# YuemingJin/STswinCL

Hardware: AMD Instinct MI355X
Metric: input frames/s, TswinPlus fwd+bwd+Adam, 4-frame 512x512 clips (higher is better)
Workload: dtype bf16; 1 GPU; BASELINE.json configs[1]: TswinPlus(12) seg train step, 4 clips/GPU x T=4 frames x 3x512x512, swin res (64,64), OHEM-CE, Adam; T=4 because the reference asserts it (swin_512.py:313); clips_per_gpu=4, frames_per_clip=4, parallelism=dp1, graph_requested=True

## Files before the change

include/stswin_hip.h:

```cpp
#ifndef STSWIN_HIP_H
#define STSWIN_HIP_H
#ifdef __cplusplus
extern "C" {
#endif

#define STSWIN_GF_GELU 1
#define STSWIN_GF_RESID 2
#define STSWIN_GF_MUL_DGELU 4
#define STSWIN_GF_OUT_F32 8
#define STSWIN_GF_ACCUM 16
#define STSWIN_GF_RELU 32
#define STSWIN_GF_MUL_R 8192
#define STSWIN_GF_C2_DGELU 16384
#define STSWIN_GF_CS_PARTIAL 32768
#define STSWIN_GF_CS_SQ 65536
#define STSWIN_GF_TAPSKIP (1 << 29)
#define STSWIN_GF_BIG 128
#define STSWIN_GF_MID 512
#define STSWIN_GF_NOPIPE 1024
#define STSWIN_GF_HALF 2048
#define STSWIN_GF_M32PP (1u << 31)
#define STSWIN_GF_W4R (1 << 30)
#define STSWIN_GF_ROT 4096
#define STSWIN_GF_NOBIG 256
// ... 181 lines not shown
                        void* out, long ldo, unsigned char* arg, int frames, int H, int W, int C, int groups, int unit_rows, void* stream);
int stswin_rows_broadcast(int dtype, const float* v, void* out, long ldo, int M, int C, int groups, float scale,
                          int accumulate, void* stream);
int stswin_bilinear(int dtype, const void* in, long ldi, void* out, long ldo, int frames, int h, int w, int H, int W, int C,
                    int backward, void* stream);
int stswin_logits_upsample(int dtype, const void* tokens, long ldt, void* nchw, int frames, int h, int w, int H, int W,
                           int nc, int backward, void* stream);

int stswin_ce_fwd(int dtype, const void* logits, const long* labels, float* loss, float* stats, int frames, long HW, int nc,
                  int ignore_index, float thresh, void* stream);
#define STSWIN_OHEM_WORK_BYTES (3 * 2048 * 12 + 48)
int stswin_ohem_select(const float* loss, long n, long n_min, float thresh, const float* stats, void* work, long work_bytes,
                       float* value, float* sel, void* stream);
int stswin_ce_bwd(int dtype, const void* logits, const long* labels, const float* loss, const float* sel,
                  const float* gscale, void* dlogits, int frames, long HW, int nc, int ignore_index, void* stream);

int stswin_contrast_fwd(int dtype, const void* Q, long ldq, const void* const* K5, long ldk, const int* lq,
                        const int* const* lk5, float* pos, float* all, int N, int HW, int C, void* stream);

int stswin_contrast_bank_fwd(int dtype, const void* Q, long ldq, const int* lq, int M, int C, int q_sets, int q_block,
                             const void* bank, long ldb, const int* lb, int maps, int seg, int bank_block, int groups,
                             const int* gmap , float inv_tau, float* pos, float* all,
                             float* rowmax, float* lse, float* workspace, long workspace_floats, void* stream);
int stswin_contrast_bank_fwd_unit(int dtype, const void* Q, long ldq, const int* lq, int M, int C, int q_sets, int q_block,
                             const void* bank, long ldb, const int* lb, int maps, int seg, int bank_block, int groups,
                             const int* gmap , float inv_tau, float* pos, float* all,
                             float* rowmax, float* lse, float* workspace, long workspace_floats, void* stream);
int stswin_contrast_class_sums(int dtype, const void* bank, long ldb, const int* lb, int maps, int seg, int bank_block, int C,
                               int ncls, float* ksum, float* scratch , void* stream);
long stswin_contrast_class_sums_scratch(int maps, int seg, int bank_block, int C, int ncls);
int stswin_contrast_bank_dq(const float* dpos, const float* dneg, const float* cnt, const int* lq, const float* ksum, float* dq,
                            long lddq, int M, int C, int q_sets, int q_block, int seg, int bank_block, int ncls, int groups, const int* gmap,
                            void* stream);

int stswin_rownorm_scatter(int dtype, const void* X, long ldx, void* Y, long ldy, float* inv, int R, int C, int views, int HW, int samples,
                           void* stream);
int stswin_rownorm_scatter_bwd(int dtype, const void* X, long ldx, const float* inv, const float* dY, long lddy, void* dX, long lddx, int R,
                               int C, int views, int HW, int samples, void* stream);
int stswin_labels_resize(const float* const* masks, int maps, int N, int Hs, int Ws, int h, int w, int* lb, void* stream);
int stswin_label_counts(const int* lq, const int* lb, int M, int maps, int seg, int q_sets, int q_block, int bank_block, int ncls, int groups,
                        const int* gmap, int* hist, float* cnt, void* stream);
int stswin_pair_loss(const float* pos, const float* all, const float* cnt, int M, int groups, int q_sets, int visible, float* loss,
                     void* stream);
int stswin_pair_loss_bwd(const float* pos, const float* all, const float* cnt, const float* dloss, int M, int groups, int q_sets, int visible,
                         float* dpos, float* dneg, void* stream);

int stswin_upsample_argmax(int dtype, const void* logits, unsigned char* labels, const long* gt, int* counts, int frames,
                           int nc, int h, int w, int H, int W, void* stream);
int stswin_upsample_argmax_cm(int dtype, const void* logits, unsigned char* labels, const long* gt, unsigned long long* cm, int ncm,
                              int align_corners, int frames, int nc, int h, int w, int H, int W, void* stream);

int stswin_frame_ingest(const unsigned char* in, unsigned char* tmp, float* out, int n, int Hs, int Ws, int H, int W,
                        const int* hbounds, const int* hcoef, int hksize, const int* vbounds, const int* vcoef, int vksize,
                        const float* lut, void* stream);
int stswin_frame_ingest_planes(const unsigned char* in, unsigned char* tmp, float* out, int n, int Hs, int Ws, int H, int W,
                               const int* hbounds, const int* hcoef, int hksize, const int* vbounds, const int* vcoef, int vksize,
                               const float* lut, void* stream);
int stswin_clip_assemble(int dtype, void* ring, const void* fresh, void* clips, const int* table, int B, int n_store, int slots,
                         int n_fresh, long frame_elems, void* stream);

long stswin_augment_crop_table_stride(int Hc, int Wc, int ksize);
int stswin_augment_crop(const unsigned char* frames, const unsigned char* labels, unsigned char* tmp, unsigned char* crop,
                        unsigned char* label_crop, const int* table, long table_stride, int ksize, int B, int T, int Hs, int Ws,
                        int Hc, int Wc, void* stream);
long stswin_augment_finish_table_stride(int Hc, int Wc);
int stswin_augment_finish(const unsigned char* crop, const unsigned char* label_crop, float* images, long* labels_out,
                          const int* table, long table_stride, const float* lut, int lut_planes, const long* label_lut, int B,
                          int T, int Hc, int Wc, void* stream);

int stswin_multi_tensor(int mode, int count, void* const* p, const void* const* g, void* const* m, void* const* v,
                        const int* n, float lr, float b1, float b2, float eps, float wd, float c1, float c2, void* stream);

int stswin_multi_tensor_lars(int count, void* const* p, const void* const* g, void* const* m, const int* n, float* norms,
                             long norms_floats, float lr, float momentum, float wd, float trust_coef, float eps, int first, int adaptive,
                             void* stream);

int stswin_optim_tick(int kind, int* counter, float* hyper, double a, double b, void* stream);
int stswin_multi_tensor_dev(int mode, int count, void* const* p, const void* const* g, void* const* m, void* const* v, const int* n,
                            const float* hyper, float b1, float b2, float eps, float wd, int first, void* stream);
int stswin_multi_tensor_lars_dev(int count, void* const* p, const void* const* g, void* const* m, const int* n, float* norms,
                                 long norms_floats, const float* hyper, float momentum, float wd, float trust_coef, float eps, int first,
                                 int adaptive, void* stream);

int stswin_selftest(float* out, int which, void* stream);
long stswin_calib_mfma(int waves_per_cu, int iters, float* sink, void* stream);
int stswin_calib_copy(const void* src, void* dst, long bytes, void* stream);
int stswin_proxy_collective(const void* src, void* dst, long bytes, int workgroups, int passes, void* stream);

#ifdef __cplusplus
}
#endif
#endif
```

stswincl_amd/csrc/optim.hip:

```cpp
#include "common.h"

#define MT_MAX 48
#define MT_CHUNK 8192

struct MTArgs {
  float* p[MT_MAX];
  const float* g[MT_MAX];
  float* m[MT_MAX];
  float* v[MT_MAX];
  int n[MT_MAX];
  int count;
  float lr, b1, b2, eps, wd, c1, c2;
  int mode;
  const float* norms;
  float trust;
  const float* hyper;
};

__global__ void optim_tick_kernel(int kind, int* __restrict__ counter, float* __restrict__ hyper, double a, double b) {
  if (threadIdx.x != 0 || blockIdx.x != 0) return;
  if (kind == 0) {
    const int t = counter[0] + 1;
    counter[0] = t;
    hyper[1] = (float)(1.0 - pow(a, (double)t));
    hyper[2] = (float)sqrt(1.0 - pow(b, (double)t));
  } else {
    const int k = counter[0];
    counter[0] = k + 1;
    hyper[3] = (float)(1.0 - (1.0 - a) * (cos(3.141592653589793 * (double)k / b) + 1.0) / 2.0);
  }
}

extern "C" int stswin_optim_tick(int kind, int* counter, float* hyper, double a, double b, void* stream) {
  if (kind < 0 || kind > 1 || !counter || !hyper) return -1604;
  hipLaunchKernelGGL(optim_tick_kernel, dim3(1), dim3(64), 0, (hipStream_t)stream, kind, counter, hyper, a, b);
  STSWIN_CHECK_LAUNCH();
  return 0;
}

__global__ __launch_bounds__(256) void mt_norms_kernel(MTArgs a, float* __restrict__ norms) {
  int b = blockIdx.x, t = 0;
  for (; t < a.count; ++t) {
    const int nb = (a.n[t] + MT_CHUNK - 1) / MT_CHUNK;
    if (b < nb) break;
    b -= nb;
  }
  if (t >= a.count) return;
  const int n = a.n[t];
  const float* __restrict__ p = a.p[t];
  const float* __restrict__ g = a.g[t];
  const int base = b * MT_CHUNK, end = min(n, base + MT_CHUNK);
  float sp = 0.f, sg = 0.f;
  for (int i = base + threadIdx.x * 4; i < end; i += 256 * 4) {
    const int cnt = min(4, end - i);
    if (cnt == 4 && ((((uintptr_t)(p + i)) | ((uintptr_t)(g + i))) & 15) == 0) {
      const f32x4 pv = *(const f32x4*)(p + i), gv = *(const f32x4*)(g + i);
#pragma unroll
      for (int e = 0; e < 4; ++e) { const float gr = gv[e] + a.wd * pv[e]; sp += pv[e] * pv[e]; sg += gr * gr; }
    } else {
      for (int e = 0; e < cnt; ++e) { const float pv = p[i + e], gr = g[i + e] + a.wd * pv; sp += pv * pv; sg += gr * gr; }
    }
  }
  sp = wave_sum(sp);
  sg = wave_sum(sg);
  __shared__ float fold[4][2];
  if ((threadIdx.x & 63) == 0) { fold[threadIdx.x >> 6][0] = sp; fold[threadIdx.x >> 6][1] = sg; }
  __syncthreads();
  if (threadIdx.x == 0) {
    norms[2 * (long)blockIdx.x] = fold[0][0] + fold[1][0] + fold[2][0] + fold[3][0];
    norms[2 * (long)blockIdx.x + 1] = fold[0][1] + fold[1][1] + fold[2][1] + fold[3][1];
  }
}

__global__ __launch_bounds__(256) void mt_norms_fold_kernel(MTArgs a, const float* __restrict__ part, float* __restrict__ norms) {
  const int t = blockIdx.x;
  long b0 = 0;
  for (int i = 0; i < t; ++i) b0 += (a.n[i] + MT_CHUNK - 1) / MT_CHUNK;
  const int nb = (a.n[t] + MT_CHUNK - 1) / MT_CHUNK;
  float sp = 0.f, sg = 0.f;
  for (int b = threadIdx.x; b < nb; b += 256) { sp += part[2 * (b0 + b)]; sg += part[2 * (b0 + b) + 1]; }
  sp = wave_sum(sp);
  sg = wave_sum(sg);
  __shared__ float fold[4][2];
  if ((threadIdx.x & 63) == 0) { fold[threadIdx.x >> 6][0] = sp; fold[threadIdx.x >> 6][1] = sg; }
  __syncthreads();
  if (threadIdx.x == 0) {
    norms[2 * t] = fold[0][0] + fold[1][0] + fold[2][0] + fold[3][0];
    norms[2 * t + 1] = fold[0][1] + fold[1][1] + fold[2][1] + fold[3][1];
  }
}

__global__ __launch_bounds__(256) void multi_tensor_kernel(MTArgs a) {
  int b = blockIdx.x, t = 0;
  for (; t < a.count; ++t) {
    const int nb = (a.n[t] + MT_CHUNK - 1) / MT_CHUNK;
    if (b < nb) break;
    b -= nb;
  }
  if (t >= a.count) return;
  const int n = a.n[t];
  float* __restrict__ p = a.p[t];
  const float* __restrict__ g = a.g[t];
  float* __restrict__ m = a.m[t];
  float* __restrict__ v = a.v[t];
  const int base = b * MT_CHUNK;
  const int end = min(n, base + MT_CHUNK);
  float lr = a.lr, b1 = a.b1, c1 = a.c1, c2 = a.c2;
  if (a.hyper) {
    if (a.mode == 2) b1 = a.hyper[3];
    else lr = a.hyper[0];
    if (a.mode == 0) { c1 = a.hyper[1]; c2 = a.hyper[2]; }
  }
  float ratio = 1.f;
  if (a.mode == 3 && a.norms) {
    const float pn = sqrtf(a.norms[2 * t]), gn = sqrtf(a.norms[2 * t + 1]);
    if (pn > 0.f && gn > 0.f) ratio = a.trust * pn / (gn + a.eps);
  }
  for (int i = base + threadIdx.x * 4; i < end; i += 256 * 4) {
    const int cnt = min(4, end - i);
    float pv[4], gv[4], mv[4], vv[4];
    const bool vec = cnt == 4 && ((((uintptr_t)(p + i)) | ((uintptr_t)(g + i))) & 15) == 0 &&
                     (a.mode == 2 || ((((uintptr_t)(m + i)) & 15) == 0 && (a.mode != 0 || (((uintptr_t)(v + i)) & 15) == 0)));
    if (vec) {
      *(f32x4*)pv = __builtin_nontemporal_load((const f32x4*)(p + i));
      *(f32x4*)gv = __builtin_nontemporal_load((const f32x4*)(g + i));
      if (a.mode != 2) *(f32x4*)mv = __builtin_nontemporal_load((const f32x4*)(m + i));
      if (a.mode == 0) *(f32x4*)vv = __builtin_nontemporal_load((const f32x4*)(v + i));
    } else {
      for (int e = 0; e < cnt; ++e) {
        pv[e] = p[i + e]; gv[e] = g[i + e];
        if (a.mode != 2) mv[e] = m[i + e];
        if (a.mode == 0) vv[e] = v[i + e];
      }
    }
#pragma unroll
    for (int e = 0; e < 4; ++e) {
      if (e >= cnt) break;
      if (a.mode == 0) {
        float gr = gv[e] + a.wd * pv[e];
        mv[e] = b1 * mv[e] + (1.f - b1) * gr;
        vv[e] = a.b2 * vv[e] + (1.f - a.b2) * gr * gr;
        const float denom = sqrtf(vv[e]) / c2 + a.eps;
        pv[e] -= (lr / c1) * (mv[e] / denom);
      } else if (a.mode == 1 || a.mode == 3) {
        float gr = (gv[e] + a.wd * pv[e]) * ratio;
        mv[e] = (c1 != 0.f) ? gr : b1 * mv[e] + gr;
        pv[e] -= lr * (b1 != 0.f ? mv[e] : gr);
      } else {
        pv[e] = pv[e] * b1 + gv[e] * (1.f - b1);
      }
    }
    if (vec) {
      __builtin_nontemporal_store(*(const f32x4*)pv, (f32x4*)(p + i));
      if (a.mode != 2) __builtin_nontemporal_store(*(const f32x4*)mv, (f32x4*)(m + i));
      if (a.mode == 0) __builtin_nontemporal_store(*(const f32x4*)vv, (f32x4*)(v + i));
    } else {
      for (int e = 0; e < cnt; ++e) {
        p[i + e] = pv[e];
        if (a.mode != 2) m[i + e] = mv[e];
        if (a.mode == 0) v[i + e] = vv[e];
      }
    }
  }
}

static int multi_tensor_impl(int mode, int count, void* const* p, const void* const* g, void* const* m, void* const* v,
                             const int* n, float lr, float b1, float b2, float eps, float wd, float c1, float c2, const float* hyper,
                             void* stream) {
  if (count <= 0) return 0;
  if (count > MT_MAX || mode < 0 || mode > 2) return -1601;
  MTArgs a;
  long blocks = 0;
  for (int i = 0; i < count; ++i) {
    a.p[i] = (float*)p[i]; a.g[i] = (const float*)g[i];
    a.m[i] = m ? (float*)m[i] : nullptr; a.v[i] = v ? (float*)v[i] : nullptr;
    a.n[i] = n[i];
    blocks += (n[i] + MT_CHUNK - 1) / MT_CHUNK;
  }
  a.count = count; a.lr = lr; a.b1 = b1; a.b2 = b2; a.eps = eps; a.wd = wd; a.c1 = c1; a.c2 = c2; a.mode = mode;
  a.norms = nullptr; a.trust = 0.f; a.hyper = hyper;
  hipLaunchKernelGGL(multi_tensor_kernel, dim3((unsigned)blocks), dim3(256), 0, (hipStream_t)stream, a);
  STSWIN_CHECK_LAUNCH();
  return 0;
}

extern "C" int stswin_multi_tensor(int mode, int count, void* const* p, const void* const* g, void* const* m, void* const* v,
                                   const int* n, float lr, float b1, float b2, float eps, float wd, float c1, float c2,
                                   void* stream) {
  return multi_tensor_impl(mode, count, p, g, m, v, n, lr, b1, b2, eps, wd, c1, c2, nullptr, stream);
}

extern "C" int stswin_multi_tensor_dev(int mode, int count, void* const* p, const void* const* g, void* const* m, void* const* v,
                                       const int* n, const float* hyper, float b1, float b2, float eps, float wd, int first,
                                       void* stream) {
  if (!hyper) return -1604;
  return multi_tensor_impl(mode, count, p, g, m, v, n, 0.f, b1, b2, eps, wd, first ? 1.f : 0.f, 1.f, hyper, stream);
}

static int multi_tensor_lars_impl(int count, void* const* p, const void* const* g, void* const* m, const int* n,
                                  float* norms, long norms_floats, float lr, const float* hyper, float momentum, float wd, float trust_coef,
                                  float eps, int first, int adaptive, void* stream) {
  if (count <= 0) return 0;
  if (count > MT_MAX || (adaptive && !norms)) return -1602;
  MTArgs a;
  long blocks = 0;
  for (int i = 0; i < count; ++i) {
    a.p[i] = (float*)p[i]; a.g[i] = (const float*)g[i]; a.m[i] = (float*)m[i]; a.v[i] = nullptr; a.n[i] = n[i];
    blocks += (n[i] + MT_CHUNK - 1) / MT_CHUNK;
  }
  a.count = count; a.lr = lr; a.b1 = momentum; a.b2 = 0.f; a.eps = eps; a.wd = wd; a.c1 = first ? 1.f : 0.f; a.c2 = 0.f; a.mode = 3;
  a.norms = adaptive ? norms : nullptr; a.trust = trust_coef; a.hyper = hyper;
  if (adaptive) {
    if (norms_floats < 2 * (long)count + 2 * blocks) return -1603;
    float* part = norms + 2 * count;
    hipLaunchKernelGGL(mt_norms_kernel, dim3((unsigned)blocks), dim3(256), 0, (hipStream_t)stream, a, part);
    hipLaunchKernelGGL(mt_norms_fold_kernel, dim3((unsigned)count), dim3(256), 0, (hipStream_t)stream, a, (const float*)part, norms);
  }
  hipLaunchKernelGGL(multi_tensor_kernel, dim3((unsigned)blocks), dim3(256), 0, (hipStream_t)stream, a);
  STSWIN_CHECK_LAUNCH();
  return 0;
}

extern "C" int stswin_multi_tensor_lars(int count, void* const* p, const void* const* g, void* const* m, const int* n,
                                        float* norms, long norms_floats, float lr, float momentum, float wd, float trust_coef, float eps,
                                        int first, int adaptive, void* stream) {
  return multi_tensor_lars_impl(count, p, g, m, n, norms, norms_floats, lr, nullptr, momentum, wd, trust_coef, eps, first, adaptive, stream);
}

extern "C" int stswin_multi_tensor_lars_dev(int count, void* const* p, const void* const* g, void* const* m, const int* n,
                                            float* norms, long norms_floats, const float* hyper, float momentum, float wd, float trust_coef,
                                            float eps, int first, int adaptive, void* stream) {
  if (!hyper) return -1604;
  return multi_tensor_lars_impl(count, p, g, m, n, norms, norms_floats, 0.f, hyper, momentum, wd, trust_coef, eps, first, adaptive, stream);
}
```

stswincl_amd/hip.py:

```python
from __future__ import annotations

import ctypes
import functools
import os
import re
from typing import Optional

import torch

_ROOT = os.path.dirname(os.path.dirname(os.path.abspath(__file__)))
LIB_PATH = os.environ.get("STSWIN_HIP_LIB") or os.path.join(_ROOT, "stswincl_amd", "lib", "libstswin_hip.so")
HEADER_PATH = os.path.join(_ROOT, "include", "stswin_hip.h")
_lib: Optional[ctypes.CDLL] = None

_c_int, _c_float, _c_void_p = ctypes.c_int, ctypes.c_float, ctypes.c_void_p


class StswinHipError(RuntimeError):
    pass


_C_TYPES = {"int": ctypes.c_int, "long": ctypes.c_long, "float": ctypes.c_float, "double": ctypes.c_double}


# ... 1245 lines not shown
    if not isinstance(t, torch.Tensor):
        raise StswinHipError(f"{fn}: {what} must be a {form}, got {type(t).__name__}")
    ok = t.is_cuda and t.dtype == dtype and t.dim() == len(shape) and t.is_contiguous() and \
        all(s is None or s == d for s, d in zip(shape, t.shape)) and (device is None or t.device == device)
    if not ok:
        raise StswinHipError(f"{fn}: {what} must be a {form}, got {t.dtype} {tuple(t.shape)} on {t.device}"
                             + ("" if t.is_contiguous() else " (not contiguous)"))
    return t


def augment_crop_table_stride(Hc: int, Wc: int, ksize: int) -> int:
    return int(load().stswin_augment_crop_table_stride(Hc, Wc, ksize))


def augment_finish_table_stride(Hc: int, Wc: int) -> int:
    return int(load().stswin_augment_finish_table_stride(Hc, Wc))


def augment_crop(frames: torch.Tensor, labels: torch.Tensor, tmp: torch.Tensor, crop: torch.Tensor, label_crop: torch.Tensor,
                 table: torch.Tensor, ksize: int):
    fn = "augment_crop"
    tensor_form(frames, torch.uint8, (None, None, None, None, 3), "frames", fn)
    B, T, Hs, Ws, _ = frames.shape
    dev = frames.device
    tensor_form(labels, torch.uint8, (B, Hs, Ws), "labels", fn, dev)
    tensor_form(crop, torch.uint8, (B, T, None, None, 3), "crop", fn, dev)
    Hc, Wc = crop.shape[2:4]
    tensor_form(label_crop, torch.uint8, (B, Hc, Wc), "label_crop", fn, dev)
    tensor_form(table, torch.int32, (B, None), "table", fn, dev)
    if table.shape[1] < augment_crop_table_stride(Hc, Wc, ksize):
        raise StswinHipError(f"{fn}: table rows must hold >= {augment_crop_table_stride(Hc, Wc, ksize)} words, got {table.shape[1]}")
    if not isinstance(tmp, torch.Tensor) or not tmp.is_cuda or tmp.dtype != torch.uint8 or not tmp.is_contiguous() or \
            tmp.numel() < B * T * Hs * Wc * 3 or tmp.device != dev:
        raise StswinHipError(f"{fn}: tmp must be contiguous uint8 on the GPU with >= {B * T * Hs * Wc * 3} bytes")
    _check(load().stswin_augment_crop(_p(frames), _p(labels), _p(tmp), _p(crop), _p(label_crop), _p(table), table.shape[1], ksize, B, T,
                                      Hs, Ws, Hc, Wc, _stream()), fn)
    return crop, label_crop


def augment_finish(crop: torch.Tensor, label_crop: torch.Tensor, images: torch.Tensor, labels_out: torch.Tensor, table: torch.Tensor,
                   lut: torch.Tensor, label_lut: torch.Tensor):
    fn = "augment_finish"
    tensor_form(crop, torch.uint8, (None, None, None, None, 3), "crop", fn)
    B, T, Hc, Wc, _ = crop.shape
    dev = crop.device
    tensor_form(label_crop, torch.uint8, (B, Hc, Wc), "label_crop", fn, dev)
    tensor_form(images, torch.float32, (B, T, 3, Hc, Wc), "images", fn, dev)
    tensor_form(labels_out, torch.int64, (B, Hc, Wc), "labels_out", fn, dev)
    tensor_form(table, torch.int32, (B, None), "table", fn, dev)
    if table.shape[1] < augment_finish_table_stride(Hc, Wc):
        raise StswinHipError(f"{fn}: table rows must hold >= {augment_finish_table_stride(Hc, Wc)} words, got {table.shape[1]}")
    tensor_form(lut, torch.float32, (3, 256) if isinstance(lut, torch.Tensor) and lut.dim() == 2 else (256,), "lut ([256] or [3][256])", fn, dev)
    tensor_form(label_lut, torch.int64, (256,), "label_lut", fn, dev)
    _check(load().stswin_augment_finish(_p(crop), _p(label_crop), _p(images), _p(labels_out), _p(table), table.shape[1], _p(lut),
                                        1 if lut.dim() == 2 else 0, _p(label_lut), B, T, Hc, Wc, _stream()), fn)
    return images, labels_out


def optim_tick(kind: int, counter: torch.Tensor, hyper: torch.Tensor, a: float, b: float) -> None:
    assert counter.dtype == torch.int32 and hyper.dtype == torch.float32 and hyper.numel() >= 4 and counter.is_cuda and hyper.is_cuda
    _check(load().stswin_optim_tick(int(kind), _p(counter), _p(hyper), a, b, _stream()), "optim_tick")


def multi_tensor(mode, ps, gs, ms=None, vs=None, lr=0.0, b1=0.0, b2=0.0, eps=0.0, wd=0.0, c1=1.0, c2=1.0, hyper=None):
    lib = load()
    st = _stream()
    for t in ps:
        if not (t.is_cuda and t.dtype == torch.float32 and t.is_contiguous()):
            raise StswinHipError("multi_tensor needs contiguous fp32 GPU tensors")
    for lo in range(0, len(ps), 48):
        hi = min(len(ps), lo + 48)
        k = hi - lo
        arr = lambda ts: (_c_void_p * k)(*[t.data_ptr() for t in ts[lo:hi]]) if ts is not None else None
        ns = (_c_int * k)(*[t.numel() for t in ps[lo:hi]])
        if hyper is not None:
            _check(lib.stswin_multi_tensor_dev(mode, k, arr(ps), arr(gs), arr(ms), arr(vs), ns, _p(hyper), b1, b2,
                                               eps, wd, 1 if (mode == 1 and c1 != 0.0) else 0, st), "multi_tensor_dev")
        else:
            _check(lib.stswin_multi_tensor(mode, k, arr(ps), arr(gs), arr(ms), arr(vs), ns, lr, b1,
                                           b2, eps, wd, c1, c2, st),
                   "multi_tensor")


def multi_tensor_lars(ps, gs, ms, norms, *, lr, momentum, wd, trust_coef, eps, first, adaptive, hyper=None):
    lib = load()
    st = _stream()
    for t in list(ps) + list(gs) + list(ms):
        if not (t.is_cuda and t.dtype == torch.float32 and t.is_contiguous()):
            raise StswinHipError("multi_tensor_lars needs contiguous fp32 GPU tensors")
    for lo in range(0, len(ps), 48):
        hi = min(len(ps), lo + 48)
        k = hi - lo
        arr = lambda ts: (_c_void_p * k)(*[t.data_ptr() for t in ts[lo:hi]])
        ns = (_c_int * k)(*[t.numel() for t in ps[lo:hi]])
        need = 2 * k + 2 * sum((t.numel() + 8191) // 8192 for t in ps[lo:hi])
        if norms is None or norms.numel() < need:
            norms = scratch(ps[lo].device, need)
        if hyper is not None:
            _check(lib.stswin_multi_tensor_lars_dev(k, arr(ps), arr(gs), arr(ms), ns, _p(norms), norms.numel(), _p(hyper),
                                                    momentum, wd, trust_coef, eps, 1 if first else 0,
                                                    1 if adaptive else 0, st), "multi_tensor_lars_dev")
            continue
        _check(lib.stswin_multi_tensor_lars(k, arr(ps), arr(gs), arr(ms), ns, _p(norms), norms.numel(), lr, momentum,
                                            wd, trust_coef, eps, 1 if first else 0,
                                            1 if adaptive else 0, st), "multi_tensor_lars")


def proxy_collective(src: torch.Tensor, dst: torch.Tensor, workgroups: int, passes: int) -> None:
    assert src.numel() * src.element_size() == dst.numel() * dst.element_size() and src.is_contiguous() and dst.is_contiguous()
    _check(load().stswin_proxy_collective(_p(src), _p(dst), src.numel() * src.element_size(), workgroups, passes, _stream()),
           "proxy_collective")


def set_cu_budget(cus: int) -> int:
    return int(load().stswin_set_cu_budget(int(cus)))


def calibrate(device=None, seconds: float = 0.1) -> dict:
    lib = load()
    dev = torch.device(device if device is not None else "cuda")
    sink = torch.zeros(4, dtype=torch.float32, device=dev)
    st = _stream()

    def timed(fn):
        a, b = torch.cuda.Event(enable_timing=True), torch.cuda.Event(enable_timing=True)
        a.record()
        fn()
        b.record()
        b.synchronize()
        return a.elapsed_time(b) * 1e-3

    iters = int(300000 * max(seconds, 0.01) / 0.1)
    per = int(lib.stswin_calib_mfma(4, 20000, _p(sink), st))
    t = min(timed(lambda: lib.stswin_calib_mfma(4, iters, _p(sink), st)) for _ in range(3))
    tflops = per * iters * 16384.0 / t / 1e12
    n = 512 << 20
    src = torch.empty(n, dtype=torch.uint8, device=dev)
    dst = torch.empty(n, dtype=torch.uint8, device=dev)
    src.zero_()
    _check(lib.stswin_calib_copy(_p(src), _p(dst), n, st), "calib_copy")
    tc = min(timed(lambda: lib.stswin_calib_copy(_p(src), _p(dst), n, st)) for _ in range(3))
    del src, dst
    return {"mfma_bf16_tflops": tflops, "mfma_probe_ms": t * 1e3, "copy_tbps": 2.0 * n / tc / 1e12, "copy_probe_ms": tc * 1e3}


def selftest(which: int) -> torch.Tensor:
    out = torch.zeros(16384, dtype=torch.float32, device="cuda")
    if which == 5:
        out[:512] = torch.arange(512, dtype=torch.float32, device="cuda")
    _check(load().stswin_selftest(_p(out), which, _stream()), "selftest")
    torch.cuda.synchronize()
    return out.cpu()
```

stswincl_amd/ops.py:

```python
from __future__ import annotations

import os
import weakref
from typing import Dict, Optional, Tuple

import torch

from . import hip

_ROWMAPS: Dict[tuple, torch.Tensor] = {}
_WCACHE: Dict[tuple, tuple] = {}


def compute_dtype(x: torch.Tensor) -> torch.dtype:
    if x.dtype == torch.bfloat16 or x.dtype == torch.float16:
        return torch.bfloat16
    if torch.is_autocast_enabled():
        return torch.bfloat16
    return torch.float32


def window_rowmap(B, T, H, W, ws, shift, device) -> torch.Tensor:
    key = ("win", B, T, H, W, ws, shift, str(device))
    m = _ROWMAPS.get(key)
    if m is None:
        m = hip.win_rowmap(B, T, H, W, ws, shift, device=device)
        _ROWMAPS[key] = m
    return m


def merge_rowmap(frames, H, W, device) -> torch.Tensor:
    key = ("merge", frames, H, W, str(device))
    m = _ROWMAPS.get(key)
    if m is None:
        m = hip.merge_rowmap(frames, H, W, device=device)
        _ROWMAPS[key] = m
    return m


def conv_rowmap(frames, H, W, dil, device) -> torch.Tensor:
    key = ("conv", frames, H, W, dil, str(device))
    m = _ROWMAPS.get(key)
    if m is None:
        m = hip.conv3x3_rowmap(frames, H, W, dil, device=device)
        _ROWMAPS[key] = m
    return m


_IDMAPS: dict = {}


def _identity_map(n: int, device) -> torch.Tensor:
    m = _IDMAPS.get((n, device))
    if m is None:
        m = torch.arange(n, dtype=torch.int32, device=device)
        _IDMAPS[(n, device)] = m
    return m


def wcast(p: torch.Tensor, dtype: torch.dtype, transpose: bool = False) -> torch.Tensor:
    key = (id(p), dtype)
    hit = _WCACHE.get(key)
    stamp = (p._version, p.data_ptr(), tuple(p.shape), p.device)
    if hit is None or hit[0]() is not p or hit[1] != stamp:
        w = p.detach()
        if (w.dim() == 2 and w.is_cuda and w.dtype == torch.float32 and dtype in (torch.bfloat16, torch.float32)
                and os.environ.get("STSWIN_TORCH_PACK") != "1"):
            n, k = w.shape
            if n % 4 == 0 and k % 4 == 0:
                fwd, tr = hip.linear_pack(w, dtype)
            else:
                fwd, tr = hip.conv_pack(w.view(n, k, 1, 1), dtype, _identity_map(n, w.device), _identity_map(k, w.device))
        else:
            fwd, tr = w.to(dtype).contiguous(), None
        if len(_WCACHE) > 4096:
            for k_ in [k_ for k_, v in _WCACHE.items() if v[0]() is None]:
                del _WCACHE[k_]
        hit = [weakref.ref(p), stamp, fwd, tr]
        _WCACHE[key] = hit
    if not transpose:
        return hit[2]
    if hit[3] is None:
        hit[3] = p.detach().t().to(dtype).contiguous()
    return hit[3]


def repack(params) -> int:
    from . import headops
    ids = {id(p): p for p in params}
    if not ids:
        return 0
    lin, conv = {}, {}
    for key, hit in _WCACHE.items():
        p = ids.get(key[0])
        if p is None or hit[0]() is not p:
            continue
        w = p.detach()
        if not (w.dim() == 2 and w.is_cuda and w.dtype == torch.float32 and w.is_contiguous() and w.shape[0] % 4 == 0
                and w.shape[1] % 4 == 0 and hit[2].shape == w.shape and hit[2].device == w.device):
            continue
        if hit[3] is not None and hit[3].shape != (w.shape[1], w.shape[0]):
            continue
        lin.setdefault(key[1], []).append((w, hit[2], hit[3]))
        hit[1] = (p._version, p.data_ptr(), tuple(p.shape), p.device)
    for key, hit in list(headops._CW.items()):
        p = ids.get(key[0])
        if p is None or hit[0]() is not p or not (p.is_cuda and p.dtype == torch.float32 and p.is_contiguous()):
            continue
        ref, _, fwd, dg, omap, imap = hit
        conv.setdefault(key[1], []).append((p.detach(), fwd, dg, omap, imap))
        headops._CW[key] = (ref, (p._version, p.data_ptr(), tuple(p.shape)), fwd, dg, omap, imap)
    n = 0
    bias = []
    for key, hit in _BIAS_TABLES.items():
        p = ids.get(key)
        if p is None or hit[0]() is not p:
            continue
        _, stamp, out, idx, umask = hit
        bias.append((p.detach(), idx, umask, out, stamp[4], stamp[5]))
        hit[1] = (p._version,) + tuple(stamp[1:])
    if bias:
        hip.bias_expand_multi(bias)
        n += len(bias)
    for dt, entries in lin.items():
        hip.linear_pack_multi(entries, dt)
        n += len(entries)
    for dt, entries in conv.items():
        hip.conv_pack_multi(entries, dt)
        n += len(entries)
    return n


def clear_caches() -> None:
    _ROWMAPS.clear()
    _PAIR_MAPS.clear()
    _COMPOSED.clear()
    _SCATTER.clear()
    _WCACHE.clear()
    _UNIQ_MASKS.clear()
    _BIAS_TABLES.clear()
    from . import headops
    headops._CW.clear()


def invalidate_weights(module: Optional[torch.nn.Module] = None) -> None:
    if module is None:
        _WCACHE.clear()
        _BIAS_TABLES.clear()
    else:
        ids = {id(p) for p in module.parameters()}
        for k in [k for k in _WCACHE if k[0] in ids]:
            del _WCACHE[k]
        for k in [k for k in _BIAS_TABLES if k in ids]:
            del _BIAS_TABLES[k]
    from . import headops
    headops._CW.clear()


def zeros_like_list(shapes, device, fill=True):
    sizes = [int(torch.Size(sh).numel()) for sh in shapes]
    offs, tot = [], 0
    for n in sizes:
        offs.append(tot)
        tot += (n + 15) // 16 * 16
    flat = hip.zeros(tot, device=device) if fill else torch.empty(tot, dtype=torch.float32, device=device)
    return [flat[o:o + n].view(sh) for o, n, sh in zip(offs, sizes, shapes)]


def wgrad_buffer(p: torch.Tensor, shape, device) -> torch.Tensor:
    from .dp import grad_dest
    d = grad_dest(p, shape) if getattr(p, "_stswin_grad_dest", None) is not None else None
    return d if d is not None else torch.empty(shape, dtype=torch.float32, device=device)


def _f32(p: Optional[torch.Tensor]) -> Optional[torch.Tensor]:
    return None if p is None else p.detach().float().contiguous()


_UNIQ_MASKS: Dict[int, tuple] = {}


_TN_GROUP = os.environ.get("STSWIN_NO_TN_GROUP") != "1"
_TN_GROUP4 = os.environ.get("STSWIN_NO_TN_GROUP4") != "1"


def _duo(site: str, M: int, N: int, K: int) -> int:
    env = os.environ.get("STSWIN_DUO")
    return hip.GF_DUO if (env and site in env.split(",")) else 0


# ... 420 lines not shown
```

stswincl_amd/optim.py:

```python
from __future__ import annotations

import math
import weakref
from typing import Iterable, Sequence

import torch

import os

from . import hip

_EAGER_REPACK = os.environ.get("STSWIN_LAZY_REPACK") != "1"


def _mark_updated(params: Sequence[torch.Tensor]) -> None:
    if not params:
        return
    setter = getattr(torch._C._autograd, "_unsafe_set_version_counter", None)
    if setter is not None:
        setter(list(params), [int(p._version) + 1 for p in params])
    else:
        torch._foreach_add_(list(params), 0)
    if _EAGER_REPACK:
        from . import ops
        ops.repack(params)


_generation = 0
_CAPTURED = weakref.WeakSet()


def bump_generation() -> None:
    global _generation
    _generation += 1


def note_captured(optimizers) -> None:
    _CAPTURED.update(optimizers)


def _refuse_in_capture(what: str, advice: str) -> None:
    if torch.cuda.is_current_stream_capturing():
        raise hip.StswinHipError(f"{what} inside a hipGraph capture: {advice}")


class _Clock:

    def __init__(self, device, step: int = 0):
        _refuse_in_capture("a new device step clock (a parameter's first gradient, the first key-encoder update, a new parameter group)",
                           "run the step eagerly once before capturing it")
        self.counter = torch.full((1,), int(step), dtype=torch.int32, device=device)
        self.hyper = torch.zeros(4, dtype=torch.float32, device=device)
        self._step, self._gen = int(step), _generation
        self.lr = None
        self.members = []

    @property
    def step(self) -> int:
        return self._step if self._gen == _generation else self.sync()

    def sync(self) -> int:
        _refuse_in_capture("a host step mirror that graph replays left stale is read", "read it before the capture")
        self._step, self._gen = int(self.counter.item()), _generation
        return self._step

    def tick(self, kind: int, a: float, b: float) -> None:
        hip.optim_tick(kind, self.counter, self.hyper, a, b)
        if self._gen == _generation:
            self._step += 1

    def load(self, step: int) -> None:
        _refuse_in_capture("a device step clock is re-seeded", "load before the capture or between replays")
        self.counter.fill_(int(step))
        self._step, self._gen = int(step), _generation

    def push_lr(self, lr: float) -> None:
        lr = float(lr)
        if self.lr != lr:
            _refuse_in_capture(f"learning rate changed ({self.lr} -> {lr})", "change it in before_step, outside the captured step")
            self.hyper[0:1].fill_(lr)
            self.lr = lr


class LrClocks:

    def __init__(self):
        self.clocks = {}

    def hyper(self, i: int, lr: float, device) -> torch.Tensor:
        c = self.clocks.get(i)
        if c is None or c.hyper.device != device:
            c = self.clocks[i] = _Clock(device)
        c.push_lr(lr)
        return c.hyper

    def push(self, param_groups) -> None:
        for i, c in self.clocks.items():
            c.push_lr(param_groups[i]["lr"])


def load_in_place(opt, state_dict, owner) -> None:
    old_state, old_groups = opt.state, opt.param_groups
    torch.optim.Optimizer.load_state_dict(opt, state_dict)
    copies, clocks, bad = [], {}, None
    for p, old in old_state.items():
        new = opt.state.get(p, {})
        for key, o in old.items():
# ... 3 lines not shown
                    clocks.setdefault(id(o), (o, []))[1].append(new)
            elif torch.is_tensor(o):
                if torch.is_tensor(v) and v.shape == o.shape and v.dtype == o.dtype and v.device == o.device:
                    copies.append((new, key, o, v))
                else:
                    bad = f"state '{key}' of a parameter loads as {None if v is None else (tuple(v.shape), v.dtype, v.device)}"
    for c, sts in clocks.values():
        if bad is None and len({int(st.get("step", -1)) for st in sts}) != 1:
            bad = "parameters that share a device clock load different step counts"
    if bad is not None:
        if owner in _CAPTURED:
            opt.state, opt.param_groups = old_state, old_groups
            raise hip.StswinHipError(f"load_state_dict after a hipGraph capture cannot be written into what the graph reads: {bad}")
        return
    for new, key, o, v in copies:
        o.copy_(v)
        new[key] = o
    for c, sts in clocks.values():
        c.load(int(sts[0]["step"]))
        c.members = sts
        for st in sts:
            st["step"], st["_clock"] = c.step, c


class FusedAdam(torch.optim.Optimizer):
    def __init__(self, params, lr=1e-3, betas=(0.9, 0.999), eps=1e-8, weight_decay=0.0):
        super().__init__(params, dict(lr=lr, betas=betas, eps=eps, weight_decay=weight_decay))
        self._gen = _generation
        self._clock_groups = []

    def _clocks(self):
        seen = {}
        for st in self.state.values():
            c = st.get("_clock")
            if c is not None:
                seen[id(c)] = c
        return list(seen.values())

    def push_hyper(self) -> None:
        for clock, i in self._clock_groups:
            clock.push_lr(self.param_groups[i]["lr"])

    def sync_steps(self) -> None:
        if self._gen != _generation:
            for c in self._clocks():
                for st in c.members:
                    st["step"] = c.step
            self._gen = _generation

    @torch.no_grad()
    def step(self, closure=None):
        loss = None
        if closure is not None:
            with torch.enable_grad():
                loss = closure()
        self.sync_steps()
        self._clock_groups = []
        for gi, group in enumerate(self.param_groups):
            b1, b2 = group["betas"]
            by_clock = {}
            touched = []
            fresh = {}
            for p in group["params"]:
                if p.grad is None:
                    continue
                st = self.state[p]
                if "exp_avg" not in st:
                    st["step"] = 0
                    st["exp_avg"] = torch.zeros_like(p, memory_format=torch.contiguous_format)
                    st["exp_avg_sq"] = torch.zeros_like(p, memory_format=torch.contiguous_format)
                if not isinstance(st["step"], int):
                    st["step"] = int(st["step"])
                clock = st.get("_clock")
                if clock is not None and clock.step != st["step"]:
                    clock = None
                if clock is None:
                    key = (st["step"], p.device)
                    clock = fresh.get(key)
                    if clock is None:
                        clock = fresh[key] = next((c for (c, *_r) in by_clock.values() if c.step == st["step"] and c.counter.device == p.device),
                                                  None) or _Clock(p.device, st["step"])
                    st["_clock"] = clock
                _c, ps, gs, ms, vs, sts = by_clock.setdefault(id(clock), (clock, [], [], [], [], []))
                ps.append(p.data)
                touched.append(p)
                gs.append(p.grad.contiguous() if not p.grad.is_contiguous() else p.grad)
                ms.append(st["exp_avg"])
                vs.append(st["exp_avg_sq"])
                sts.append(st)
            for clock, ps, gs, ms, vs, sts in by_clock.values():
                self._clock_groups.append((clock, gi))
                clock.push_lr(group["lr"])
                clock.tick(0, float(b1), float(b2))
                clock.members = sts
                for st in sts:
                    st["step"] = clock.step
                hip.multi_tensor(0, ps, gs, ms, vs, b1=b1, b2=b2, eps=group["eps"], wd=group["weight_decay"], hyper=clock.hyper)
            _mark_updated(touched)
        return loss

    def state_dict(self):
        self.sync_steps()
        sd = super().state_dict()
        sd["state"] = {k: {kk: vv for kk, vv in v.items() if kk != "_clock"} for k, v in sd["state"].items()}
        return sd

    def load_state_dict(self, state_dict):
        self.sync_steps()
        load_in_place(self, state_dict, self)
        for st in self.state.values():
            if "step" in st and not isinstance(st["step"], int):
                st["step"] = int(st["step"])


class FusedSGD(torch.optim.Optimizer):
    def __init__(self, params, lr=1e-3, momentum=0.0, weight_decay=0.0):
        super().__init__(params, dict(lr=lr, momentum=momentum, weight_decay=weight_decay))
        self._lr = LrClocks()

    def push_hyper(self) -> None:
        self._lr.push(self.param_groups)

    def load_state_dict(self, state_dict):
        load_in_place(self, state_dict, self)

    @torch.no_grad()
    def step(self, closure=None):
        loss = None
        if closure is not None:
            with torch.enable_grad():
                loss = closure()
        for gi, group in enumerate(self.param_groups):
            first, later, touched = ([], [], []), ([], [], []), []
            for p in group["params"]:
                if p.grad is None:
                    continue
                st = self.state[p]
                g = p.grad.contiguous() if not p.grad.is_contiguous() else p.grad
                if st.get("momentum_buffer") is None:
                    st["momentum_buffer"] = torch.zeros_like(p, memory_format=torch.contiguous_format)
                    tgt = first
                else:
                    tgt = later
                tgt[0].append(p.data)
                touched.append(p)
                tgt[1].append(g)
                tgt[2].append(st["momentum_buffer"])
            for (ps, gs, ms), c1 in ((first, 1.0), (later, 0.0)):
                if ps:
                    hip.multi_tensor(1, ps, gs, ms, None, b1=group["momentum"], wd=group["weight_decay"], c1=c1,
                                     hyper=self._lr.hyper(gi, group["lr"], ps[0].device))
            _mark_updated(touched)
        return loss


@torch.no_grad()
def ema_update(keys: Sequence[torch.Tensor], queries: Sequence[torch.Tensor], momentum: float, hyper=None) -> None:
    hip.multi_tensor(2, [k.data for k in keys], [q.data for q in queries], b1=momentum, hyper=hyper)
    _mark_updated(list(keys))


class EmaSchedule:

    def __init__(self, device, base_momentum: float, K: int, k: int = 0):
        self.clock = _Clock(device, k)
        self.m0, self.K = float(base_momentum), float(K)

    def tick(self) -> torch.Tensor:
        self.clock.tick(1, self.m0, self.K)
        return self.clock.hyper

    @property
    def k(self) -> int:
        return self.clock.step

    def sync(self) -> int:
        return self.clock.sync()


def make_contrast_optimizer(params, batch_size: int, base_learning_rate: float = 1.0, momentum: float = 0.9,
                            weight_decay: float = 1e-5, optimizer: str = "lars"):
# ... 9 lines not shown
```

Before: 627.3 frames/s.

## Fuse Adam update with bf16 weight repacking into one kernel

Adds a fused multi-tensor Adam kernel that, for linear and conv weights with cached bf16 packed copies, writes the bf16 forward and transposed/permuted layouts directly from the freshly updated fp32 values via an LDS tile. This removes the separate repack pass that re-reads the fp32 weights after the optimizer step, and the Python path restamps the caches instead of repacking them. Other parameters still use the old multi-tensor kernel. The cost is a more complex kernel with scattered single-element bf16 stores for conv maps, plus a host-side map check that runs once per cache entry.

Result: no change. 628.0 frames/s, median of 4 (+0.1%).

```diff
diff --git a/include/stswin_hip.h b/include/stswin_hip.h
--- a/include/stswin_hip.h
+++ b/include/stswin_hip.h
@@ -287,6 +287,11 @@
                                  long norms_floats, const float* hyper, float momentum, float wd, float trust_coef, float eps, int first,
                                  int adaptive, void* stream);
 
+int stswin_multi_tensor_pack_dev(int dtype, int count, void* const* p, const void* const* g, void* const* m, void* const* v,
+                                 void* const* fwd, void* const* tr, const int* const* omap, const int* const* imap, const int* d0,
+                                 const int* d1, const int* S, const int* cop, const int* cip, const float* hyper, float b1, float b2,
+                                 float eps, float wd, void* stream);
+
 int stswin_selftest(float* out, int which, void* stream);
 long stswin_calib_mfma(int waves_per_cu, int iters, float* sink, void* stream);
 int stswin_calib_copy(const void* src, void* dst, long bytes, void* stream);
diff --git a/stswincl_amd/csrc/optim.hip b/stswincl_amd/csrc/optim.hip
--- a/stswincl_amd/csrc/optim.hip
+++ b/stswincl_amd/csrc/optim.hip
@@ -90,6 +90,23 @@
   }
 }
 
+DEVI void adam_elem(float& p, float g, float& m, float& v, float lr, float b1, float b2, float eps, float wd, float c1, float c2) {
+  float gr = g + wd * p;
+  m = b1 * m + (1.f - b1) * gr;
+  v = b2 * v + (1.f - b2) * gr * gr;
+  const float denom = sqrtf(v) / c2 + eps;
+  p -= (lr / c1) * (m / denom);
+}
+
+DEVI void adam_vec4(f32x4& p, const f32x4 g, f32x4& m, f32x4& v, float lr, float b1, float b2, float eps, float wd, float c1, float c2) {
+#pragma unroll
+  for (int e = 0; e < 4; ++e) {
+    float pe = p[e], me = m[e], ve = v[e];
+    adam_elem(pe, g[e], me, ve, lr, b1, b2, eps, wd, c1, c2);
+    p[e] = pe; m[e] = me; v[e] = ve;
+  }
+}
+
 __global__ __launch_bounds__(256) void multi_tensor_kernel(MTArgs a) {
   int b = blockIdx.x, t = 0;
   for (; t < a.count; ++t) {
@@ -137,11 +154,7 @@
     for (int e = 0; e < 4; ++e) {
       if (e >= cnt) break;
       if (a.mode == 0) {
-        float gr = gv[e] + a.wd * pv[e];
-        mv[e] = b1 * mv[e] + (1.f - b1) * gr;
-        vv[e] = a.b2 * vv[e] + (1.f - a.b2) * gr * gr;
-        const float denom = sqrtf(vv[e]) / c2 + a.eps;
-        pv[e] -= (lr / c1) * (mv[e] / denom);
+        adam_elem(pv[e], gv[e], mv[e], vv[e], lr, b1, a.b2, a.eps, a.wd, c1, c2);
       } else if (a.mode == 1 || a.mode == 3) {
         float gr = (gv[e] + a.wd * pv[e]) * ratio;
         mv[e] = (c1 != 0.f) ? gr : b1 * mv[e] + gr;
@@ -197,6 +210,211 @@
   return multi_tensor_impl(mode, count, p, g, m, v, n, 0.f, b1, b2, eps, wd, first ? 1.f : 0.f, 1.f, hyper, stream);
 }
 
+#define MTP_MAX 40
+#define MTP_LDS_BYTES 18496
+struct MTPArgs {
+  float* p[MTP_MAX]; const float* g[MTP_MAX]; float* m[MTP_MAX]; float* v[MTP_MAX];
+  bf16* fwd[MTP_MAX];
+  bf16* tr[MTP_MAX];
+  const int* omap[MTP_MAX]; const int* imap[MTP_MAX];
+  int d0[MTP_MAX], d1[MTP_MAX];
+  int S[MTP_MAX];
+  int cop[MTP_MAX], cip[MTP_MAX], tiles[MTP_MAX];
+  int count;
+  float b1, b2, eps, wd;
+  const float* hyper;
+};
+
+static_assert(sizeof(MTPArgs) < 4096, "kernel arguments stay below 4 KB");
+
+static __host__ __device__ inline int mtp_conv_ot(int S) {
+  int ot = 64;
+  while (ot > 0 && (long)ot * (64 * S + 2) * 2 > MTP_LDS_BYTES) ot >>= 1;
+  return ot;
+}
+
+template <bool NT> DEVI void mtp_store4(bf16* dst, const f32x4 v) {
+  const bf16x4 o = {(bf16)v[0], (bf16)v[1], (bf16)v[2], (bf16)v[3]};
+  if (NT) __builtin_nontemporal_store(__builtin_bit_cast(short4v, o), (short4v*)dst);
+  else *(bf16x4*)dst = o;
+}
+template <bool NT> DEVI void mtp_store1(bf16* dst, const bf16 o) {
+  if (NT) __builtin_nontemporal_store(__builtin_bit_cast(short, o), (short*)dst);
+  else *dst = o;
+}
+
+template <bool NT>
+__global__ __launch_bounds__(256) void multi_tensor_pack_kernel(MTPArgs a) {
+  __shared__ __attribute__((aligned(16))) unsigned char lds[MTP_LDS_BYTES];
+  __shared__ int s_opos[64], s_ipos[64];
+  int b = blockIdx.x, t = 0;
+  for (; t < a.count; ++t) {
+    if (b < a.tiles[t]) break;
+    b -= a.tiles[t];
+  }
+  if (t >= a.count) return;
+  float* __restrict__ p = a.p[t];
+  const float* __restrict__ g = a.g[t];
+  float* __restrict__ m = a.m[t];
+  float* __restrict__ v = a.v[t];
+  bf16* __restrict__ fwd = a.fwd[t];
+  bf16* __restrict__ tr = a.tr[t];
+  const float lr = a.hyper[0], c1 = a.hyper[1], c2 = a.hyper[2];
+  const float b1 = a.b1, b2 = a.b2, eps = a.eps, wd = a.wd;
+  const int S = a.S[t];
+  if (S == 0) {
+    const int n = a.d0[t], k = a.d1[t], tk = (k + 63) / 64;
+    const int k0 = (b % tk) * 64, n0 = (b / tk) * 64;
+    float (*tile)[65] = (float (*)[65])lds;
+    const int gq = threadIdx.x & 15, r = threadIdx.x >> 4;
+    f32x4 pv[4], gv[4], mv[4], vv[4];
+#pragma unroll
+    for (int ps = 0; ps < 4; ++ps) {
+      const int gn = n0 + ps * 16 + r, gk = k0 + gq * 4;
+      pv[ps] = (f32x4){0.f, 0.f, 0.f, 0.f};
+      if (gn < n && gk < k) {
+        const long i = (long)gn * k + gk;
+        pv[ps] = __builtin_nontemporal_load((const f32x4*)(p + i));
+        gv[ps] = __builtin_nontemporal_load((const f32x4*)(g + i));
+        mv[ps] = __builtin_nontemporal_load((const f32x4*)(m + i));
+        vv[ps] = __builtin_nontemporal_load((const f32x4*)(v + i));
+      }
+    }
+#pragma unroll
+    for (int ps = 0; ps < 4; ++ps) {
+      const int row = ps * 16 + r, gn = n0 + row, gk = k0 + gq * 4;
+      if (gn < n && gk < k) {
+        const long i = (long)gn * k + gk;
+        adam_vec4(pv[ps], gv[ps], mv[ps], vv[ps], lr, b1, b2, eps, wd, c1, c2);
+        __builtin_nontemporal_store(pv[ps], (f32x4*)(p + i));
+        __builtin_nontemporal_store(mv[ps], (f32x4*)(m + i));
+        __builtin_nontemporal_store(vv[ps], (f32x4*)(v + i));
+        mtp_store4<NT>(fwd + i, pv[ps]);
+      }
+#pragma unroll
+      for (int e = 0; e < 4; ++e) tile[row][gq * 4 + e] = pv[ps][e];
+    }
+    if (!tr) return;
+    __syncthreads();
+#pragma unroll
+    for (int ps = 0; ps < 4; ++ps) {
+      const int row = ps * 16 + r, gk = k0 + row, gn = n0 + gq * 4;
+      if (gk < k && gn < n)
+        mtp_store4<NT>(tr + (long)gk * n + gn, (f32x4){tile[gq * 4 + 0][row], tile[gq * 4 + 1][row], tile[gq * 4 + 2][row], tile[gq * 4 + 3][row]});
+    }
+    return;
+  }
+  const int co = a.d0[t], ci = a.d1[t], cop = a.cop[t], cip = a.cip[t];
+  const int OT = mtp_conv_ot(S), LROW = 64 * S + 2, to = (co + OT - 1) / OT;
+  const int so0 = (b % to) * OT, si0 = (b / to) * 64;
+  const int ot = min(OT, co - so0), it = min(64, ci - si0);
+  bf16* T = (bf16*)lds;
+  if (threadIdx.x < 64) s_opos[threadIdx.x] = -1;
+  else if (threadIdx.x < 128) s_ipos[threadIdx.x - 64] = -1;
+  __syncthreads();
+  {
+    const int* __restrict__ omap = a.omap[t];
+    const int* __restrict__ imap = a.imap[t];
+    for (int pos = threadIdx.x; pos < cop; pos += 256) { const int src = omap[pos] - so0; if (src >= 0 && src < ot) s_opos[src] = pos; }
+    for (int pos = threadIdx.x; pos < cip; pos += 256) { const int src = imap[pos] - si0; if (src >= 0 && src < it) s_ipos[src] = pos; }
+  }
+  const int nv = it * S / 4, total = ot * nv;
+  for (int q0 = threadIdx.x; q0 < total; q0 += 512) {
+    long i[2];
+    int lo[2];
+    f32x4 pv[2], gv[2], mv[2], vv[2];
+#pragma unroll
+    for (int u = 0; u < 2; ++u) {
+      const int q = q0 + u * 256;
+      if (q < total) {
+        const int ol = q / nv, vi = q - ol * nv;
+        i[u] = ((long)(so0 + ol) * ci + si0) * S + vi * 4;
+        lo[u] = ol * LROW + vi * 4;
+        pv[u] = __builtin_nontemporal_load((const f32x4*)(p + i[u]));
+        gv[u] = __builtin_nontemporal_load((const f32x4*)(g + i[u]));
+        mv[u] = __builtin_nontemporal_load((const f32x4*)(m + i[u]));
+        vv[u] = __builtin_nontemporal_load((const f32x4*)(v + i[u]));
+      }
+    }
+#pragma unroll
+    for (int u = 0; u < 2; ++u) {
+      if (q0 + u * 256 < total) {
+        adam_vec4(pv[u], gv[u], mv[u], vv[u], lr, b1, b2, eps, wd, c1, c2);
+        __builtin_nontemporal_store(pv[u], (f32x4*)(p + i[u]));
+        __builtin_nontemporal_store(mv[u], (f32x4*)(m + i[u]));
+        __builtin_nontemporal_store(vv[u], (f32x4*)(v + i[u]));
+        bf16x2* d = (bf16x2*)(T + lo[u]);
+        d[0] = (bf16x2){(bf16)pv[u][0], (bf16)pv[u][1]};
+        d[1] = (bf16x2){(bf16)pv[u][2], (bf16)pv[u][3]};
+      }
+    }
+  }
+  __syncthreads();
+  {
+    const int il = threadIdx.x & 63, ipos = il < it ? s_ipos[il] : -1;
+    if (ipos >= 0)
+      for (int r = threadIdx.x >> 6; r < ot * S; r += 4) {
+        const int ol = r / S, s = r - ol * S, opos = s_opos[ol];
+        if (opos >= 0) mtp_store1<NT>(fwd + ((long)opos * S + s) * cip + ipos, T[ol * LROW + il * S + s]);
+      }
+  }
+  if (!tr) return;
+  {
+    const int ol = threadIdx.x & (OT - 1), opos = ol < ot ? s_opos[ol] : -1;
+    if (opos >= 0)
+      for (int r = threadIdx.x / OT; r < it * S; r += 256 / OT) {
+        const int il = r / S, s = r - il * S, ipos = s_ipos[il];
+        if (ipos >= 0) mtp_store1<NT>(tr + ((long)ipos * S + s) * cop + opos, T[ol * LROW + r]);
+      }
+  }
+}
+
+extern "C" int stswin_multi_tensor_pack_dev(int dtype, int count, void* const* p, const void* const* g, void* const* m, void* const* v,
+                                            void* const* fwd, void* const* tr, const int* const* omap, const int* const* imap,
+                                            const int* d0, const int* d1, const int* S, const int* cop, const int* cip,
+                                            const float* hyper, float b1, float b2, float eps, float wd, void* stream) {
+  if (dtype != 0) return -1605;
+  if (count <= 0) return 0;
+  if (!hyper || !p || !g || !m || !v || !fwd || !d0 || !d1 || !S) return -1604;
+  for (int i = 0; i < count; ++i) {
+    if (!p[i] || !g[i] || !m[i] || !v[i] || !fwd[i]) return -1604;
+    if ((((uintptr_t)p[i]) | ((uintptr_t)g[i]) | ((uintptr_t)m[i]) | ((uintptr_t)v[i])) & 15) return -1606;
+    if ((((uintptr_t)fwd[i]) | ((uintptr_t)(tr ? tr[i] : nullptr))) & 7) return -1606;
+    if (d0[i] <= 0 || d1[i] <= 0 || S[i] < 0 || d1[i] % 4 || (S[i] == 0 && d0[i] % 4)) return -1607;
+    if (S[i] > 0) {
+      if (!omap || !imap || !cop || !cip || !omap[i] || !imap[i] || cop[i] <= 0 || cip[i] <= 0 || mtp_conv_ot(S[i]) < 1) return -1607;
+      if ((long)((d0[i] + mtp_conv_ot(S[i]) - 1) / mtp_conv_ot(S[i])) * ((d1[i] + 63) / 64) > 0x7fffffffL) return -1607;
+    } else if ((long)((d0[i] + 63) / 64) * ((d1[i] + 63) / 64) > 0x7fffffffL) return -1607;
+  }
+  static const bool plain = [] { const char* e = getenv("STSWIN_ADAM_PACK_PLAIN_STORES"); return e && e[0] == '1'; }();
+  for (int lo = 0; lo < count; lo += MTP_MAX) {
+    const int c = count - lo < MTP_MAX ? count - lo : MTP_MAX;
+    MTPArgs a;
+    long blocks = 0;
+    for (int j = 0; j < c; ++j) {
+      const int i = lo + j;
+      a.p[j] = (float*)p[i]; a.g[j] = (const float*)g[i]; a.m[j] = (float*)m[i]; a.v[j] = (float*)v[i];
+      a.fwd[j] = (bf16*)fwd[i]; a.tr[j] = tr ? (bf16*)tr[i] : nullptr;
+      a.d0[j] = d0[i]; a.d1[j] = d1[i]; a.S[j] = S[i];
+      if (S[i] > 0) {
+        const int ot = mtp_conv_ot(S[i]);
+        a.omap[j] = omap[i]; a.imap[j] = imap[i]; a.cop[j] = cop[i]; a.cip[j] = cip[i];
+        a.tiles[j] = ((d0[i] + ot - 1) / ot) * ((d1[i] + 63) / 64);
+      } else {
+        a.omap[j] = a.imap[j] = nullptr; a.cop[j] = a.cip[j] = 0;
+        a.tiles[j] = ((d0[i] + 63) / 64) * ((d1[i] + 63) / 64);
+      }
+      blocks += a.tiles[j];
+    }
+    if (blocks > 0x7fffffffL) return -1607;
+    a.count = c; a.b1 = b1; a.b2 = b2; a.eps = eps; a.wd = wd; a.hyper = hyper;
+    if (plain) hipLaunchKernelGGL(multi_tensor_pack_kernel<false>, dim3((unsigned)blocks), dim3(256), 0, (hipStream_t)stream, a);
+    else hipLaunchKernelGGL(multi_tensor_pack_kernel<true>, dim3((unsigned)blocks), dim3(256), 0, (hipStream_t)stream, a);
+    STSWIN_CHECK_LAUNCH();
+  }
+  return 0;
+}
+
 static int multi_tensor_lars_impl(int count, void* const* p, const void* const* g, void* const* m, const int* n,
                                   float* norms, long norms_floats, float lr, const float* hyper, float momentum, float wd, float trust_coef,
                                   float eps, int first, int adaptive, void* stream) {
diff --git a/stswincl_amd/hip.py b/stswincl_amd/hip.py
--- a/stswincl_amd/hip.py
+++ b/stswincl_amd/hip.py
@@ -1351,6 +1351,25 @@
                    "multi_tensor")
 
 
+def multi_tensor_pack(entries, *, hyper, b1, b2, eps, wd):
+    if not entries:
+        return
+    c = len(entries)
+    for e in entries:
+        for t in e[:4]:
+            if not (t.is_cuda and t.dtype == torch.float32 and t.is_contiguous()):
+                raise StswinHipError("multi_tensor_pack needs contiguous fp32 GPU tensors")
+        if e[4].dtype != torch.bfloat16 or (e[5] is not None and e[5].dtype != torch.bfloat16):
+            raise StswinHipError("multi_tensor_pack writes bf16 operands only")
+    arr = lambda i: (_c_void_p * c)(*[(e[i].data_ptr() if e[i] is not None else 0) for e in entries])
+    ints = lambda f: (_c_int * c)(*[f(e) for e in entries])
+    conv = lambda e: e[6] is not None
+    _check(load().stswin_multi_tensor_pack_dev(
+        0, c, arr(0), arr(1), arr(2), arr(3), arr(4), arr(5), arr(6), arr(7), ints(lambda e: e[0].shape[0]), ints(lambda e: e[0].shape[1]),
+        ints(lambda e: e[0].shape[2] * e[0].shape[3] if conv(e) else 0), ints(lambda e: e[6].numel() if conv(e) else 0),
+        ints(lambda e: e[7].numel() if conv(e) else 0), _p(hyper), b1, b2, eps, wd, _stream()), "multi_tensor_pack_dev")
+
+
 def multi_tensor_lars(ps, gs, ms, norms, *, lr, momentum, wd, trust_coef, eps, first, adaptive, hyper=None):
     lib = load()
     st = _stream()
diff --git a/stswincl_amd/ops.py b/stswincl_amd/ops.py
--- a/stswincl_amd/ops.py
+++ b/stswincl_amd/ops.py
@@ -85,6 +85,70 @@
     return hit[3]
 
 
+def _lin_batchable(p: torch.Tensor, hit) -> bool:
+    w = p.detach()
+    return (w.dim() == 2 and w.is_cuda and w.dtype == torch.float32 and w.is_contiguous() and w.shape[0] % 4 == 0
+            and w.shape[1] % 4 == 0 and hit[2].shape == w.shape and hit[2].device == w.device
+            and (hit[3] is None or hit[3].shape == (w.shape[1], w.shape[0])))
+
+
+def _conv_batchable(p: torch.Tensor) -> bool:
+    return p.is_cuda and p.dtype == torch.float32 and p.is_contiguous()
+
+
+_MAP_ONCE: dict = {}
+
+
+def _map_names_each_once(m: torch.Tensor, channels: int) -> bool:
+    hit = _MAP_ONCE.get((id(m), channels))
+    if hit is None or hit[0]() is not m:
+        if torch.cuda.is_current_stream_capturing():
+            return False
+        v = m.detach().cpu()
+        v = v[v >= 0].sort().values
+        hit = (weakref.ref(m), bool(v.numel() == channels and torch.equal(v, torch.arange(channels, dtype=v.dtype))))
+        _MAP_ONCE[(id(m), channels)] = hit
+    return hit[1]
+
+
+def adam_pack_targets(params) -> dict:
+    from . import headops
+    ids = {id(p): p for p in params}
+    found: dict = {}
+    if not ids:
+        return found
+    for key, hit in _WCACHE.items():
+        p = ids.get(key[0])
+        if p is None or hit[0]() is not p:
+            continue
+        ok = key[1] == torch.bfloat16 and key[0] not in found and _lin_batchable(p, hit)
+        found[key[0]] = (hit[2], hit[3], None, None) if ok else None
+    for key, hit in headops._CW.items():
+        p = ids.get(key[0])
+        if p is None or hit[0]() is not p:
+            continue
+        _, _, fwd, dg, omap, imap = hit
+        ok = (key[1] == torch.bfloat16 and key[0] not in found and _conv_batchable(p) and p.dim() == 4 and p.shape[1] % 4 == 0
+              and p.shape[2] * p.shape[3] <= 144 and _map_names_each_once(omap, p.shape[0]) and _map_names_each_once(imap, p.shape[1]))
+        found[key[0]] = (fwd, dg, omap, imap) if ok else None
+    return {k: v for k, v in found.items() if v is not None}
+
+
+def restamp(params) -> None:
+    from . import headops
+    ids = {id(p): p for p in params}
+    if not ids:
+        return
+    for key, hit in _WCACHE.items():
+        p = ids.get(key[0])
+        if p is not None and hit[0]() is p:
+            hit[1] = (p._version, p.data_ptr(), tuple(p.shape), p.device)
+    for key, hit in list(headops._CW.items()):
+        p = ids.get(key[0])
+        if p is not None and hit[0]() is p:
+            headops._CW[key] = (hit[0], (p._version, p.data_ptr(), tuple(p.shape))) + tuple(hit[2:])
+
+
 def repack(params) -> int:
     from . import headops
     ids = {id(p): p for p in params}
@@ -96,16 +160,13 @@
         if p is None or hit[0]() is not p:
             continue
         w = p.detach()
-        if not (w.dim() == 2 and w.is_cuda and w.dtype == torch.float32 and w.is_contiguous() and w.shape[0] % 4 == 0
-                and w.shape[1] % 4 == 0 and hit[2].shape == w.shape and hit[2].device == w.device):
-            continue
-        if hit[3] is not None and hit[3].shape != (w.shape[1], w.shape[0]):
+        if not _lin_batchable(p, hit):
             continue
         lin.setdefault(key[1], []).append((w, hit[2], hit[3]))
         hit[1] = (p._version, p.data_ptr(), tuple(p.shape), p.device)
     for key, hit in list(headops._CW.items()):
         p = ids.get(key[0])
-        if p is None or hit[0]() is not p or not (p.is_cuda and p.dtype == torch.float32 and p.is_contiguous()):
+        if p is None or hit[0]() is not p or not _conv_batchable(p):
             continue
         ref, _, fwd, dg, omap, imap = hit
         conv.setdefault(key[1], []).append((p.detach(), fwd, dg, omap, imap))
diff --git a/stswincl_amd/optim.py b/stswincl_amd/optim.py
--- a/stswincl_amd/optim.py
+++ b/stswincl_amd/optim.py
@@ -13,7 +13,11 @@
 _EAGER_REPACK = os.environ.get("STSWIN_LAZY_REPACK") != "1"
 
 
-def _mark_updated(params: Sequence[torch.Tensor]) -> None:
+def _adam_pack() -> bool:
+    return os.environ.get("STSWIN_ADAM_PACK") != "0"
+
+
+def _mark_updated(params: Sequence[torch.Tensor], packed: Sequence[torch.Tensor] = ()) -> None:
     if not params:
         return
     setter = getattr(torch._C._autograd, "_unsafe_set_version_counter", None)
@@ -21,8 +25,12 @@
         setter(list(params), [int(p._version) + 1 for p in params])
     else:
         torch._foreach_add_(list(params), 0)
+    from . import ops
+    if packed:
+        ops.restamp(packed)
+        done = {id(p) for p in packed}
+        params = [p for p in params if id(p) not in done]
     if _EAGER_REPACK:
-        from . import ops
         ops.repack(params)
 
 
@@ -192,12 +200,16 @@
                                                   None) or _Clock(p.device, st["step"])
                     st["_clock"] = clock
                 _c, ps, gs, ms, vs, sts = by_clock.setdefault(id(clock), (clock, [], [], [], [], []))
-                ps.append(p.data)
+                ps.append(p)
                 touched.append(p)
                 gs.append(p.grad.contiguous() if not p.grad.is_contiguous() else p.grad)
                 ms.append(st["exp_avg"])
                 vs.append(st["exp_avg_sq"])
                 sts.append(st)
+            targets, packed = {}, []
+            if _adam_pack():
+                from . import ops
+                targets = ops.adam_pack_targets(touched)
             for clock, ps, gs, ms, vs, sts in by_clock.values():
                 self._clock_groups.append((clock, gi))
                 clock.push_lr(group["lr"])
@@ -205,8 +217,20 @@
                 clock.members = sts
                 for st in sts:
                     st["step"] = clock.step
-                hip.multi_tensor(0, ps, gs, ms, vs, b1=b1, b2=b2, eps=group["eps"], wd=group["weight_decay"], hyper=clock.hyper)
-            _mark_updated(touched)
+                fused, plain = [], ([], [], [], [])
+                for p, g, m, v in zip(ps, gs, ms, vs):
+                    tgt = targets.get(id(p))
+                    if tgt is not None and (p.data_ptr() | g.data_ptr() | m.data_ptr() | v.data_ptr()) % 16 == 0:
+                        fused.append((p.data, g, m, v) + tgt)
+                        packed.append(p)
+                    else:
+                        for lst, t in zip(plain, (p.data, g, m, v)):
+                            lst.append(t)
+                kw = dict(b1=b1, b2=b2, eps=group["eps"], wd=group["weight_decay"], hyper=clock.hyper)
+                hip.multi_tensor_pack(fused, **kw)
+                if plain[0]:
+                    hip.multi_tensor(0, *plain, **kw)
+            _mark_updated(touched, packed)
         return loss
 
     def state_dict(self):
```
